# Shreyas2409/Rust-Image-Transform

Measured on AMD Instinct MI355X. Metric: transform MPix/s (decode+resize+encode) 4096²→512² WebP q80; 1/2/4/8 GPU, higher is better.
Workload: dtype u8

## Files before the change

rust-image-transform_amd/csrc/ik_png.hip:

```cpp
#include <algorithm>
#include <cstdlib>
#include <cstring>
#include <type_traits>

#include "ik_crc.h"
#include "ik_inflate.h"
#include "ik_internal.h"
#include "ik_png.h"
#include "ik_png_wave.h"
#include "ik_unfilter.h"

namespace ik {

__device__ __forceinline__ void raise_priority() { __builtin_amdgcn_s_setprio(3); }

typedef __attribute__((address_space(3))) uint32_t lds_word;
struct FindWin {
    const IK_GLOBAL uint32_t* W;
    uint64_t wend;
    lds_word* win;
    uint32_t r0;
    __device__ void fetch(uint64_t base) {
        if (base + 32 > wend + 64) {
            for (int k = 0; k < 32; ++k) win[64 * k] = base + k < wend ? W[base + k] : 0u;
// ... 1294 lines not shown
                const int i = __builtin_ctz(mk);
                mk &= mk - 1u;
                if (k < (uint32_t)kResolveList) {
                    s_pos[k++] = (uint32_t)(x0 + i);
                    continue;
                }
                const int rv = infl::resolve_at(I.u16, I.obase, I.nlanes, I.page_lane, kPngPageShift, e0 + i);
                if (rv < 0) atomicOr(err + ir.x, 2);
                o[i >> 2] = (o[i >> 2] & ~(255u << (8 * (i & 3)))) | (((uint32_t)rv & 255u) << (8 * (i & 3)));
            }
        }
        *reinterpret_cast<IK_GLOBAL uint4*>(drow + x0) = make_uint4(o[0], o[1], o[2], o[3]);
    }
    __syncthreads();
    const uint32_t cnt = s_cnt < (uint32_t)kResolveList ? s_cnt : (uint32_t)kResolveList;
    const int64_t hlo = s_hlo, hhi = s_hhi;
    for (uint32_t m = threadIdx.x; m < cnt; m += 256) {
        const uint32_t x = s_pos[m];
        const int64_t q = rs + 1 + (int64_t)x;
        int rv;
        if (q >= hlo && q < hhi) {
            const uint32_t mv = I.u16[q];
            const int64_t q2 = hlo - infl::kWindow + (int64_t)(mv & 0x7FFFu);
            rv = (mv & 0x8000u) && q2 >= 0 ? infl::resolve_at(I.u16, I.obase, I.nlanes, I.page_lane, kPngPageShift, q2) : -1;
        } else {
            rv = infl::resolve_at(I.u16, I.obase, I.nlanes, I.page_lane, kPngPageShift, q);
        }
        if (rv < 0) atomicOr(err + ir.x, 2);
        drow[x] = (uint8_t)rv;
    }
}

__device__ __forceinline__ uint32_t wave_shr1(uint32_t v, uint32_t lane0) {
    return (uint32_t)__builtin_amdgcn_update_dpp((int)lane0, (int)v, 0x138, 0xF, 0xF, false);
}

__device__ __forceinline__ uint32_t byte_of(const uint32_t (&w)[4], int i) { return (w[i >> 2] >> (8 * (i & 3))) & 255u; }

typedef unsigned u32x4 __attribute__((ext_vector_type(4)));
constexpr int kUnfG = 8;

typedef const __attribute__((address_space(1))) u32x4* gu32x4p;
constexpr int kCpolSc1 = 16;

__device__ __forceinline__ uint64_t uniform_u64(uint64_t v) {
    const uint32_t lo = (uint32_t)__builtin_amdgcn_readfirstlane((int)(uint32_t)v);
    const uint32_t hi = (uint32_t)__builtin_amdgcn_readfirstlane((int)(uint32_t)(v >> 32));
    return ((uint64_t)hi << 32) | lo;
}

struct FtMask {
    uint32_t sub, up, avg, paeth;
    __device__ explicit FtMask(uint32_t ft)
        : sub(ft == 1 ? ~0u : 0u), up(ft == 2 ? ~0u : 0u), avg(ft == 3 ? ~0u : 0u), paeth(ft == 4 ? ~0u : 0u) {}
};

template <int BPP, bool SWAR = false>
__device__ __forceinline__ void unfilter_chunk(const u32x4& rawv, const uint32_t (&up)[4], const uint32_t (&prevup)[4],
                                               const uint32_t (&prevcur)[4], const FtMask& fm, uint32_t (&o)[4]) {
    const uint32_t raw[4] = {rawv.x, rawv.y, rawv.z, rawv.w};
    if constexpr (SWAR && (BPP == 4 || BPP == 8)) {
        constexpr int K = BPP / 4;
#pragma unroll
        for (int k = 0; k < 4; ++k) {
            const uint32_t a = k >= K ? o[k - K] : prevcur[4 + k - K];
            const uint32_t c = k >= K ? up[k - K] : prevup[4 + k - K];
            o[k] = unfilter_word(raw[k], a, up[k], c, fm.sub, fm.up, fm.avg, fm.paeth);
        }
        return;
    }
    o[0] = o[1] = o[2] = o[3] = 0;
#pragma unroll
    for (int i = 0; i < 16; ++i) {
        const uint32_t a = i >= BPP ? ((o[(i - BPP) >> 2] >> (8 * ((i - BPP) & 3))) & 255u)
                                    : byte_of(prevcur, 16 + i - BPP);
        const uint32_t b = byte_of(up, i);
        const uint32_t c = i >= BPP ? byte_of(up, i - BPP) : byte_of(prevup, 16 + i - BPP);
        const int d1 = (int)b - (int)c, d2 = (int)a - (int)c;
        const int pa = d1 < 0 ? -d1 : d1, pb = d2 < 0 ? -d2 : d2, pc = (d1 + d2) < 0 ? -(d1 + d2) : (d1 + d2);
        const uint32_t paeth = (pa <= pb && pa <= pc) ? a : (pb <= pc ? b : c);
        const uint32_t pred = (a & fm.sub) | (b & fm.up) | (((a + b) >> 1) & fm.avg) | (paeth & fm.paeth);
        const uint32_t v = (byte_of(raw, i) + pred) & 255u;
        o[i >> 2] |= v << (8 * (i & 3));
    }
}

#ifdef IK_UNF_PROF
__device__ unsigned long long g_unf_prof[8];
hipError_t png_unf_prof_read(unsigned long long* out) {
    hipError_t e = hipMemcpyFromSymbol(out, HIP_SYMBOL(g_unf_prof), sizeof(g_unf_prof));
    unsigned long long z[8] = {};
    if (e == hipSuccess) e = hipMemcpyToSymbol(HIP_SYMBOL(g_unf_prof), z, sizeof(z));
    return e;
}
#define IK_UNF_T(k) do { const unsigned long long _t = clock64(); up_[k] += _t - t_; t_ = _t; } while (0)
#else
#define IK_UNF_T(k) do { } while (0)
#endif

template <int BPP, bool SWAR>
__global__ __launch_bounds__(kPngUnfilterThreads) void k_png_unfilter(const PngImgDev* imgs, const int2* groups,
                                                                      const int* prog_base, unsigned* prog,
                                                                      unsigned* ticket) {
    raise_priority();
    constexpr int NW = kPngUnfilterThreads / 64, G = kUnfG;
    __shared__ int s_t;
    if (threadIdx.x == 0) s_t = (int)atomicAdd(ticket, 1u);
    __syncthreads();
    const int2 gk = groups[s_t];
    const PngImgDev I = imgs[gk.x];
    if (png_unfilter_scan_path(BPP, I.rowbytes, *(const volatile int*)I.flags)) return;
    const int wave = __builtin_amdgcn_readfirstlane(threadIdx.x >> 6), lane = threadIdx.x & 63;
    const int nch = (I.rowbytes + 15) >> 4;
    const int nbands = (I.H + 63) >> 6;
    const int K = png_unfilter_groups(I.H);
    unsigned* pg = prog + prog_base[gk.x];
#ifdef IK_UNF_PROF
    unsigned long long up_[6] = {0, 0, 0, 0, 0, 0}, t_ = clock64();
#endif
    for (int band = wave * K + gk.y; band < nbands; band += NW * K) {
        const int y = band * 64 + lane;
        const bool live = y < I.H;
        const FtMask fm(live ? I.ft[y] : 0u);
        const bool above = band > 0;
        uint32_t cur[4] = {0, 0, 0, 0}, up[4] = {0, 0, 0, 0};
        uint32_t prevcur[4] = {0, 0, 0, 0}, prevup[4] = {0, 0, 0, 0};
        const uint64_t dbase = uniform_u64((uint64_t)(size_t)I.dst);
        const size_t ibytes = I.pitch * (size_t)I.H;
        const __amdgpu_buffer_rsrc_t rs = __builtin_amdgcn_make_buffer_rsrc(
            (void*)dbase, (short)0, (int)(ibytes < 0x7fffffffu ? ibytes : 0x7fffffffu), 0x00020000);
        const uint32_t rowoff = (uint32_t)((size_t)(live ? y : 0) * I.pitch);
        auto fetch = [&](int s0, u32x4 (&r)[G]) {
#pragma unroll
            for (int t = 0; t < G; ++t) {
                const uint32_t off = rowoff + 16u * (uint32_t)min(max(s0 + t - lane, 0), nch - 1);
                r[t] = __builtin_bit_cast(u32x4, __builtin_amdgcn_raw_buffer_load_b128(rs, (int)off, 0, 0));
            }
        };
        unsigned seen = 0;
        const int ngrp = (nch + 63 + G - 1) / G;
        auto group = [&](int g, u32x4 (&rc)[G], u32x4 (&rn)[G]) {
            const int s0 = g * G;
            u32x4 ab[G];
#pragma unroll
            for (int t = 0; t < G; ++t) ab[t] = u32x4{0, 0, 0, 0};
            IK_UNF_T(0);
            if (above && s0 < nch) {
                const unsigned need = (unsigned)min(s0 + G, nch);
                while (seen < need) {
                    const unsigned v = __hip_atomic_load(pg + band - 1, __ATOMIC_RELAXED, __HIP_MEMORY_SCOPE_AGENT);
                    seen = (unsigned)__builtin_amdgcn_readfirstlane((int)v);
                    if (seen < need) __builtin_amdgcn_s_sleep(1);
                }
                const uint32_t aoff = lane == 0 ? (uint32_t)((size_t)(band * 64 - 1) * I.pitch) : 0x80000000u;
#pragma unroll
                for (int t = 0; t < G; ++t)
                    ab[t] = __builtin_bit_cast(u32x4, __builtin_amdgcn_raw_buffer_load_b128(
                                                          rs, (int)(aoff + 16u * (uint32_t)min(s0 + t, nch - 1)), 0, kCpolSc1));
            }
            IK_UNF_T(1);
            if (g + 1 < ngrp) fetch(s0 + G, rn);
#pragma unroll
            for (int t = 0; t < G; ++t) {
                const int j = s0 + t - lane;
                uint32_t nup[4];
                nup[0] = wave_shr1(cur[0], ab[t].x);
                nup[1] = wave_shr1(cur[1], ab[t].y);
                nup[2] = wave_shr1(cur[2], ab[t].z);
                nup[3] = wave_shr1(cur[3], ab[t].w);
                const bool act = live && j >= 0 && j < nch;
                if (act) {
#pragma unroll
                    for (int k = 0; k < 4; ++k) { prevup[k] = up[k]; up[k] = nup[k]; prevcur[k] = cur[k]; }
                    if (j == 0) {
#pragma unroll
                        for (int k = 0; k < 4; ++k) { prevup[k] = 0; prevcur[k] = 0; }
                    }
                    uint32_t o[4];
                    unfilter_chunk<BPP, SWAR>(rc[t], up, prevup, prevcur, fm, o);
#pragma unroll
                    for (int k = 0; k < 4; ++k) cur[k] = o[k];
                }
                const u32x4 ov = {cur[0], cur[1], cur[2], cur[3]};
                __builtin_amdgcn_raw_buffer_store_b128(__builtin_bit_cast(__attribute__((ext_vector_type(4))) unsigned, ov),
                                                       rs, (int)(act ? rowoff + 16u * (uint32_t)j : 0x80000000u), 0,
                                                       kCpolSc1);
            }
            IK_UNF_T(2);
            const int jl = s0 + G - 1 - 63;
            if (jl >= 0 && band * 64 + 63 < I.H) {
                asm volatile("s_waitcnt vmcnt(0)" ::: "memory");
                if (lane == 63)
                    __hip_atomic_store(pg + band, (unsigned)min(jl + 1, nch), __ATOMIC_RELAXED, __HIP_MEMORY_SCOPE_AGENT);
            }
            IK_UNF_T(3);
        };
        u32x4 ra[G], rb[G];
        fetch(0, ra);
        for (int g = 0; g < ngrp; g += 2) {
            group(g, ra, rb);
            if (g + 1 < ngrp) group(g + 1, rb, ra);
        }
    }
#ifdef IK_UNF_PROF
    if (lane == 0) {
        for (int k = 0; k < 5; ++k) atomicAdd(&g_unf_prof[k], up_[k]);
        atomicAdd(&g_unf_prof[7], 1ull);
    }
#endif
}

__device__ __forceinline__ uint32_t add_bytes(uint32_t a, uint32_t b) {
    return ((a & 0x7F7F7F7Fu) + (b & 0x7F7F7F7Fu)) ^ ((a ^ b) & 0x80808080u);
}
__device__ __forceinline__ uint32_t wave_scan_bytes(uint32_t v) {
    v = add_bytes(v, (uint32_t)__builtin_amdgcn_update_dpp(0, (int)v, 0x111, 0xF, 0xF, true));
    v = add_bytes(v, (uint32_t)__builtin_amdgcn_update_dpp(0, (int)v, 0x112, 0xF, 0xF, true));
    v = add_bytes(v, (uint32_t)__builtin_amdgcn_update_dpp(0, (int)v, 0x114, 0xF, 0xF, true));
    v = add_bytes(v, (uint32_t)__builtin_amdgcn_update_dpp(0, (int)v, 0x118, 0xF, 0xF, true));
    const uint32_t r0 = (uint32_t)__builtin_amdgcn_readlane((int)v, 15);
    const uint32_t r1 = add_bytes(r0, (uint32_t)__builtin_amdgcn_readlane((int)v, 31));
    const uint32_t r2 = add_bytes(r1, (uint32_t)__builtin_amdgcn_readlane((int)v, 47));
    const int row = (int)(threadIdx.x & 63) >> 4;
    return add_bytes(v, row == 0 ? 0u : row == 1 ? r0 : row == 2 ? r1 : r2);
}

template <int CH>
__global__ __launch_bounds__(kSuThreads) void k_png_unfilter_su(const PngImgDev* imgs, int nimg) {
    raise_priority();
    constexpr int kSuChunks = CH;
    __shared__ uint32_t s_w[kSuThreads / 64];
    typedef uint32_t u4 __attribute__((ext_vector_type(4)));
    const int im = (int)blockIdx.x / kSuRanges, jr = (int)blockIdx.x % kSuRanges;
    if (im >= nimg) return;
    const PngImgDev I = imgs[im];
    if (!png_unfilter_scan_path(4, I.rowbytes, *(const volatile int*)I.flags)) return;
    const int H = I.H, nch = (I.rowbytes + 15) >> 4;
    if ((nch <= kSuThreads * ::ik::kSuChunks) != (CH == ::ik::kSuChunks)) return;
    const int tid = threadIdx.x, wv = tid >> 6;
    const int c0 = tid * kSuChunks;
    const int y1 = (int)((int64_t)H * (jr + 1) / kSuRanges);
    int y = (int)((int64_t)H * jr / kSuRanges);
    const IK_GLOBAL uint8_t* ft = (const IK_GLOBAL uint8_t*)I.ft;
    while (y < y1 && y != 0 && ft[y] > 1) ++y;
    while (y < y1) {
        uint32_t prev[4 * kSuChunks];
#pragma unroll
        for (int k = 0; k < 4 * kSuChunks; ++k) prev[k] = 0;
        int r = y;
        do {
            const uint32_t f = ft[r];
            IK_GLOBAL uint8_t* row = (IK_GLOBAL uint8_t*)(I.dst + (size_t)r * I.pitch);
            uint32_t w[4 * kSuChunks];
#pragma unroll
            for (int i = 0; i < kSuChunks; ++i) {
                const u4 v = c0 + i < nch ? *(const IK_GLOBAL u4*)(row + 16 * (c0 + i)) : u4{0, 0, 0, 0};
                w[4 * i] = v.x; w[4 * i + 1] = v.y; w[4 * i + 2] = v.z; w[4 * i + 3] = v.w;
            }
            if (f == 2) {
#pragma unroll
                for (int k = 0; k < 4 * kSuChunks; ++k) w[k] = add_bytes(w[k], prev[k]);
            } else if (f == 1) {
#pragma unroll
                for (int k = 1; k < 4 * kSuChunks; ++k) w[k] = add_bytes(w[k], w[k - 1]);
                const uint32_t incl = wave_scan_bytes(w[4 * kSuChunks - 1]);
                uint32_t carry = (uint32_t)__builtin_amdgcn_update_dpp(0, (int)incl, 0x138, 0xF, 0xF, true);
                if ((tid & 63) == 63) s_w[wv] = incl;
                __syncthreads();
                for (int q = 0; q < wv; ++q) carry = add_bytes(carry, s_w[q]);
                __syncthreads();
#pragma unroll
                for (int k = 0; k < 4 * kSuChunks; ++k) w[k] = add_bytes(w[k], carry);
            }
#pragma unroll
            for (int i = 0; i < kSuChunks; ++i)
                if (c0 + i < nch) *(IK_GLOBAL u4*)(row + 16 * (c0 + i)) = u4{w[4 * i], w[4 * i + 1], w[4 * i + 2], w[4 * i + 3]};
#pragma unroll
            for (int k = 0; k < 4 * kSuChunks; ++k) prev[k] = w[k];
            ++r;
        } while (r < H && ft[r] == 2);
        y = r;
    }
}

hipError_t launch_png_unfilter_su(const PngImgDev* imgs, int nimg, hipStream_t s) {
    if (nimg <= 0) return hipSuccess;
    hipLaunchKernelGGL(k_png_unfilter_su<kSuChunks>, dim3(nimg * kSuRanges), dim3(kSuThreads), 0, s, imgs, nimg);
    hipLaunchKernelGGL(k_png_unfilter_su<kSuChunksWide>, dim3(nimg * kSuRanges), dim3(kSuThreads), 0, s, imgs, nimg);
    return hipGetLastError();
}

__global__ __launch_bounds__(256) void k_copy_words(const uint32_t* __restrict__ src, uint32_t* __restrict__ dst,
                                                    size_t n) {
    for (size_t i = (size_t)blockIdx.x * 256 + threadIdx.x; i < n; i += (size_t)gridDim.x * 256) dst[i] = src[i];
}

hipError_t launch_copy_words(const uint32_t* src, uint32_t* dst, size_t n, hipStream_t s) {
    if (!n) return hipSuccess;
    const size_t blocks = std::min<size_t>((n + 255) / 256, 1024);
    hipLaunchKernelGGL(k_copy_words, dim3((unsigned)blocks), dim3(256), 0, s, src, dst, n);
    return hipGetLastError();
}

struct CrcOps {
    uint32_t x2n[32];
    uint32_t level[8];
    uint32_t piece;
    uint32_t crc_idat;
};

__global__ __launch_bounds__(256) void k_png_gather(uintptr_t raw, uint8_t* __restrict__ stream,
                                                    const PngGatherPiece* __restrict__ pieces,
                                                    uint32_t* __restrict__ piece_crc, CrcOps ops) {
    __shared__ uint32_t t[1024];
    __shared__ uint32_t s_crc[256], s_len[256];
    const int tid = (int)threadIdx.x;
    t[tid] = crc::table_entry((uint32_t)tid);
    __syncthreads();
#pragma unroll
    for (int sl = 1; sl < 4; ++sl) {
        const uint32_t prev = t[256 * (sl - 1) + tid];
        t[256 * sl + tid] = (prev >> 8) ^ t[prev & 255u];
        __syncthreads();
    }
    const PngGatherPiece P = pieces[blockIdx.x];
    const uint32_t b0 = 256u * (uint32_t)tid;
    const uint32_t len = P.len > b0 ? (P.len - b0 < 256u ? P.len - b0 : 256u) : 0u;
    uint32_t c = ~0u;
    IK_GLOBAL uint8_t* dp = (IK_GLOBAL uint8_t*)(stream + P.dst + b0);
    if (len && P.src == kPngNoSrc) {
        for (uint32_t i = 0; i < len; ++i) dp[i] = 0;
    } else if (len) {
        const IK_GLOBAL uint8_t* sp = (const IK_GLOBAL uint8_t*)(raw + (uintptr_t)(P.src + b0));
        uint32_t i = 0;
        const uint32_t mis = (uint32_t)((uintptr_t)dp & 3u);
        const uint32_t pre = mis ? (4u - mis < len ? 4u - mis : len) : 0u;
        for (; i < pre; ++i) {
            const uint32_t b = sp[i];
            dp[i] = (uint8_t)b;
            c = crc::step_byte(c, b, t);
        }
        const uint32_t nw = (len - i) >> 2;
        if (nw) {
            const uintptr_t sa = (uintptr_t)(sp + i);
            const uint32_t sh = (uint32_t)(sa & 3u);
            const IK_GLOBAL uint32_t* ws = reinterpret_cast<const IK_GLOBAL uint32_t*>(sa - sh);
            IK_GLOBAL uint32_t* wd = reinterpret_cast<IK_GLOBAL uint32_t*>(dp + i);
            uint32_t lo = ws[0];
            uint32_t k = 0;
            for (; k + 8 <= nw; k += 8) {
                uint32_t in[9];
                in[0] = lo;
#pragma unroll
                for (int u = 1; u <= 8; ++u) in[u] = sh ? ws[k + u] : (u < 8 ? ws[k + u] : 0u);
#pragma unroll
                for (int u = 0; u < 8; ++u) {
                    const uint32_t v = sh ? __builtin_amdgcn_alignbyte(in[u + 1], in[u], sh) : in[u];
                    wd[k + u] = v;
                    c = crc::step_word(c, v, t);
                }
                lo = sh ? in[8] : (k + 8 < nw ? ws[k + 8] : 0u);
            }
            for (; k < nw; ++k) {
                const uint32_t hi = sh ? ws[k + 1] : 0u;
                const uint32_t v = sh ? __builtin_amdgcn_alignbyte(hi, lo, sh) : lo;
                wd[k] = v;
                c = crc::step_word(c, v, t);
                lo = sh ? hi : (k + 1 < nw ? ws[k + 1] : 0u);
            }
            i += 4u * nw;
        }
        for (; i < len; ++i) {
            const uint32_t b = sp[i];
            dp[i] = (uint8_t)b;
            c = crc::step_byte(c, b, t);
        }
    }
    s_crc[tid] = ~c;
    s_len[tid] = len;
    __syncthreads();
#pragma unroll 1
    for (int k = 0; k < 8; ++k) {
        const int stride = 1 << k;
        if ((tid & (2 * stride - 1)) == 0) {
            const uint32_t rl = s_len[tid + stride];
            if (rl) {
                const uint32_t op = rl == (256u << k) ? ops.level[k] : crc::x8n(rl, ops.x2n);
                s_crc[tid] = crc::combine_op(s_crc[tid], s_crc[tid + stride], op);
                s_len[tid] += rl;
            }
        }
        __syncthreads();
    }
    if (tid == 0) {
        piece_crc[2 * blockIdx.x] = s_crc[0];
        piece_crc[2 * blockIdx.x + 1] = s_len[0];
    }
}

__global__ __launch_bounds__(256) void k_png_crc_check(uintptr_t raw,
                                                       const PngCrcChunk* __restrict__ chunks, int nchunks,
                                                       const uint32_t* __restrict__ piece_crc, int* err, CrcOps ops) {
    const int i = (int)(blockIdx.x * blockDim.x + threadIdx.x);
    if (i >= nchunks) return;
    const PngCrcChunk C = chunks[i];
    uint32_t c = ops.crc_idat;
    for (uint32_t p = C.piece0; p < C.piece0 + C.npieces; ++p) {
        const uint32_t len = piece_crc[2 * p + 1];
        const uint32_t op = len == kPngGatherPiece ? ops.piece : crc::x8n(len, ops.x2n);
        c = crc::combine_op(c, piece_crc[2 * p], op);
    }
    const IK_GLOBAL uint8_t* q = (const IK_GLOBAL uint8_t*)(raw + (uintptr_t)C.crc_at);
    const uint32_t stored = (uint32_t)q[0] << 24 | (uint32_t)q[1] << 16 | (uint32_t)q[2] << 8 | (uint32_t)q[3];
    if (c != stored) err[C.stream] = 1;
}

static CrcOps crc_ops() {
    static const CrcOps o = [] {
        CrcOps r{};
        crc::x2n_table(r.x2n);
        for (int k = 0; k < 8; ++k) r.level[k] = crc::x8n((uint64_t)256 << k, r.x2n);
        r.piece = crc::x8n(kPngGatherPiece, r.x2n);
        uint32_t t[1024];
        for (uint32_t i = 0; i < 256; ++i) t[i] = crc::table_entry(i);
        for (int sl = 1; sl < 4; ++sl)
            for (int i = 0; i < 256; ++i) t[256 * sl + i] = (t[256 * (sl - 1) + i] >> 8) ^ t[t[256 * (sl - 1) + i] & 255u];
        uint32_t c = ~0u;
        for (const char ch : {'I', 'D', 'A', 'T'}) c = crc::step_byte(c, (uint8_t)ch, t);
        r.crc_idat = ~c;
        return r;
    }();
    return o;
}

hipError_t launch_png_gather(uintptr_t raw, uint8_t* stream, const PngGatherPiece* pieces, int npieces,
                             uint32_t* piece_crc, hipStream_t s) {
    if (npieces <= 0) return hipSuccess;
    hipLaunchKernelGGL(k_png_gather, dim3((unsigned)npieces), dim3(256), 0, s, raw, stream, pieces, piece_crc,
                       crc_ops());
    return hipGetLastError();
}

hipError_t launch_png_crc_check(uintptr_t raw, const PngCrcChunk* chunks, int nchunks, const uint32_t* piece_crc,
                                int* err, hipStream_t s) {
    if (nchunks <= 0) return hipSuccess;
    hipLaunchKernelGGL(k_png_crc_check, dim3((unsigned)((nchunks + 255) / 256)), dim3(256), 0, s, raw, chunks,
                       nchunks, piece_crc, err, crc_ops());
    return hipGetLastError();
}

__global__ __launch_bounds__(64) void k_png_walk(const uint64_t* __restrict__ files, const uint64_t* __restrict__ lens,
                                                 PngWalkRec* __restrict__ recs, uint8_t* __restrict__ side,
                                                 int* __restrict__ out_n) {
    const int f = (int)blockIdx.x, lane = (int)threadIdx.x;
    const IK_GLOBAL uint8_t* b = (const IK_GLOBAL uint8_t*)(uintptr_t)files[f];
    const uint64_t n = lens[f];
    PngWalkRec* R = recs + (size_t)f * kPngWalkRecs;
    uint8_t* S = side + (size_t)f * kPngWalkSide;
    uint64_t pos = 8;
    uint32_t used = 0;
    int cnt = 0, st = 0;
    while (pos + 12 <= n) {
        uint8_t h[12];
#pragma unroll
        for (int k = 0; k < 12; ++k) h[k] = b[pos + k];
        const uint32_t len = (uint32_t)h[0] << 24 | (uint32_t)h[1] << 16 | (uint32_t)h[2] << 8 | h[3];
        if ((uint64_t)len > n - pos - 12) { st = -3; break; }
        if (cnt == kPngWalkRecs) { st = -1; break; }
        const bool idat = h[4] == 'I' && h[5] == 'D' && h[6] == 'A' && h[7] == 'T';
        uint32_t so = ~0u;
        if (!idat || !len) {
            if (used + len + 8 > kPngWalkSide) { st = -2; break; }
            so = used;
            for (uint32_t i = (uint32_t)lane; i < len + 8; i += 64) S[so + i] = b[pos + 4 + i];
            used += (len + 8 + 3) & ~3u;
        }
        if (lane == 0) {
            PngWalkRec r;
            r.off = pos;
            r.len = len;
            r.side = so;
#pragma unroll
            for (int k = 0; k < 4; ++k) { r.type[k] = h[4 + k]; r.head[k] = h[8 + k]; }
            R[cnt] = r;
        }
        ++cnt;
        pos += 12 + (uint64_t)len;
        if (h[4] == 'I' && h[5] == 'E' && h[6] == 'N' && h[7] == 'D') break;
    }
    if (lane == 0) out_n[f] = st ? st : cnt;
}

__global__ __launch_bounds__(64) void k_copy_heads(const uint64_t* __restrict__ files, const uint64_t* __restrict__ lens,
                                                   uint8_t* __restrict__ out) {
    const int f = (int)blockIdx.x, t = (int)threadIdx.x;
    const IK_GLOBAL uint8_t* b = (const IK_GLOBAL uint8_t*)(uintptr_t)files[f];
    out[64 * (size_t)f + t] = (uint64_t)t < lens[f] ? b[t] : 0;
}

hipError_t launch_copy_heads(const uint64_t* files, const uint64_t* lens, int n, uint8_t* out, hipStream_t s) {
    if (n <= 0) return hipSuccess;
    hipLaunchKernelGGL(k_copy_heads, dim3((unsigned)n), dim3(64), 0, s, files, lens, out);
    return hipGetLastError();
}

hipError_t launch_png_walk(const uint64_t* files, const uint64_t* lens, int n, PngWalkRec* recs, uint8_t* side,
                           int* out_n, hipStream_t s) {
    if (n <= 0) return hipSuccess;
    hipLaunchKernelGGL(k_png_walk, dim3((unsigned)n), dim3(64), 0, s, files, lens, recs, side, out_n);
    return hipGetLastError();
}

__device__ __forceinline__ int a7_pass(uint32_t xr, int yr) {
    if (yr & 1) return 6;
    if (xr & 1) return 5;
    if (yr & 2) return 4;
    if (xr & 2) return 3;
    if (yr & 4) return 2;
    return (xr & 4) ? 1 : 0;
}

template <int BITS>
__device__ __forceinline__ void a7_row(const PngA7Dev& I, int y, uint32_t seg, uint8_t* lds) {
    constexpr int UB = BITS == 24 || BITS == 48 ? 48 : 16;
    constexpr uint32_t SEG = kA7Threads * UB;
    typedef uint32_t u4 __attribute__((ext_vector_type(4)));
    const uint32_t tid = threadIdx.x;
    const size_t ub = (size_t)seg * SEG + (size_t)tid * UB;
    IK_GLOBAL uint8_t* const drow = (IK_GLOBAL uint8_t*)(I.dst + (size_t)y * I.pitch);
    if (y & 1) {
        const IK_GLOBAL uint8_t* srow = (const IK_GLOBAL uint8_t*)(I.pass[6].src + (size_t)(y >> 1) * I.pass[6].pitch);
#pragma unroll
        for (int c = 0; c < UB / 16; ++c)
            if (ub + 16 * c < (size_t)I.rowbytes) *(IK_GLOBAL u4*)(drow + ub + 16 * c) = *(const IK_GLOBAL u4*)(srow + ub + 16 * c);
        return;
    }
    const int yr = y & 7;
#pragma unroll
    for (int p = 0; p < 6; ++p) {
        const int ldx = 3 - (p >> 1), ldy = p < 3 ? 3 : p < 5 ? 2 : 1, y0 = p == 2 ? 4 : p == 4 ? 2 : 0;
        if ((yr - y0) & ((1 << ldy) - 1)) continue;
        const uint32_t len = SEG >> ldx, ro = (p & 1) ? len : 0u;
        const size_t s0 = ((size_t)seg * SEG) >> ldx;
        const IK_GLOBAL uint8_t* srow = (const IK_GLOBAL uint8_t*)(I.pass[p].src + (size_t)(y >> ldy) * I.pass[p].pitch);
        for (uint32_t b = tid * 16; b < len; b += kA7Threads * 16) {
            u4 v = {0, 0, 0, 0};
            if (I.pass[p].src && s0 + b < (size_t)I.pass[p].rowbytes) v = *(const IK_GLOBAL u4*)(srow + s0 + b);
            *reinterpret_cast<u4*>(lds + ro + b) = v;
        }
    }
    __syncthreads();
    uint32_t o[UB / 4];
#pragma unroll
    for (int k = 0; k < UB / 4; ++k) o[k] = 0;
    if constexpr (BITS >= 8) {
        constexpr int BPP = BITS / 8, NPX = UB / BPP;
        constexpr int E = BPP % 4 == 0 ? 4 : BPP % 2 == 0 ? 2 : 1;
#pragma unroll
        for (int i = 0; i < NPX; ++i) {
            const uint32_t xl = tid * NPX + i;
            const int p = a7_pass(xl & 7u, yr), ldx = 3 - (p >> 1);
            const uint32_t a = ((p & 1) ? SEG >> ldx : 0u) + (xl >> ldx) * BPP;
#pragma unroll
            for (int k = 0; k < BPP / E; ++k) {
                const int pos = i * BPP + k * E;
                uint32_t v;
                if constexpr (E == 4) v = *reinterpret_cast<const uint32_t*>(lds + a + 4 * k);
                else if constexpr (E == 2) v = *reinterpret_cast<const uint16_t*>(lds + a + 2 * k);
                else v = lds[a + k];
                o[pos >> 2] |= v << (8 * (pos & 3));
            }
        }
    } else {
        constexpr int F = 8 / BITS;
#pragma unroll
        for (int j = 0; j < 16; ++j) {
            uint32_t byte = 0;
#pragma unroll
            for (int f = 0; f < F; ++f) {
                const uint32_t xl = (tid * 16 + j) * F + f;
                const int p = a7_pass(xl & 7u, yr), ldx = 3 - (p >> 1);
                const uint32_t sb = (xl >> ldx) * BITS;
                const uint32_t v = ((uint32_t)lds[((p & 1) ? SEG >> ldx : 0u) + (sb >> 3)] >> (8 - BITS - (sb & 7u))) & ((1u << BITS) - 1u);
                byte |= v << (8 - BITS - f * BITS);
            }
            o[j >> 2] |= byte << (8 * (j & 3));
        }
    }
#pragma unroll
    for (int c = 0; c < UB / 16; ++c)
        if (ub + 16 * c < (size_t)I.rowbytes)
            *(IK_GLOBAL u4*)(drow + ub + 16 * c) = u4{o[4 * c], o[4 * c + 1], o[4 * c + 2], o[4 * c + 3]};
}

__global__ __launch_bounds__(kA7Threads) void k_png_adam7(const PngA7Dev* imgs, int n) {
    raise_priority();
    __shared__ __attribute__((aligned(16))) uint8_t s_run[kA7Threads * 48];
    int lo = 0, hi = n - 1;
    while (lo < hi) {
        const int mid = (lo + hi + 1) >> 1;
        if (imgs[mid].blk0 <= blockIdx.x) lo = mid;
        else hi = mid - 1;
    }
    const PngA7Dev& I = imgs[lo];
    const uint32_t r = blockIdx.x - I.blk0;
    const int y = (int)(r / I.nseg);
    const uint32_t seg = r % I.nseg;
    if (y >= I.h) return;
    switch (I.bits) {
    case 1: a7_row<1>(I, y, seg, s_run); break;
    case 2: a7_row<2>(I, y, seg, s_run); break;
    case 4: a7_row<4>(I, y, seg, s_run); break;
    case 8: a7_row<8>(I, y, seg, s_run); break;
    case 16: a7_row<16>(I, y, seg, s_run); break;
    case 24: a7_row<24>(I, y, seg, s_run); break;
    case 32: a7_row<32>(I, y, seg, s_run); break;
    case 48: a7_row<48>(I, y, seg, s_run); break;
    case 64: a7_row<64>(I, y, seg, s_run); break;
    default: break;
    }
}

hipError_t launch_png_adam7(const PngA7Dev* imgs, int n, uint32_t nblocks, hipStream_t s) {
    if (n <= 0 || !nblocks) return hipSuccess;
    hipLaunchKernelGGL(k_png_adam7, dim3(nblocks), dim3(kA7Threads), 0, s, imgs, n);
    return hipGetLastError();
}

__global__ __launch_bounds__(256) void k_png_px(PngPxDev P) {
    __shared__ uint32_t pal[256];
    if (P.ctype == 3) pal[threadIdx.x] = P.pal[threadIdx.x];
    __syncthreads();
    const int x = (int)(blockIdx.x * 256 + threadIdx.x), y = (int)blockIdx.y;
    if (x >= P.w) return;
    const uint8_t* r = P.src + (size_t)y * P.sp;
    if (P.depth == 16) {
        const int spp = P.ctype == 0 ? 1 : P.ctype == 2 ? 3 : P.ctype == 4 ? 2 : 4;
        const uint8_t* s = r + (size_t)2 * spp * x;
        uint16_t* o16 = reinterpret_cast<uint16_t*>(P.dst + (size_t)y * P.dp) + (size_t)x * P.out_c;
        bool key = P.out_c > spp;
#pragma unroll 4
        for (int k = 0; k < spp; ++k) {
            const int v = (int)s[2 * k] << 8 | s[2 * k + 1];
            o16[k] = (uint16_t)v;
            key = key && v == (P.ctype == 0 ? P.key : P.key_rgb[k]);
        }
        if (P.out_c > spp) o16[spp] = key ? 0 : 65535;
        return;
    }
    uint8_t* o = P.dst + (size_t)y * P.dp + (size_t)x * P.out_c;
    if (P.ctype == 2) {
        const int R = r[3 * x], G = r[3 * x + 1], B = r[3 * x + 2];
        o[0] = (uint8_t)R; o[1] = (uint8_t)G; o[2] = (uint8_t)B;
        o[3] = (R == P.key_rgb[0] && G == P.key_rgb[1] && B == P.key_rgb[2]) ? 0 : 255;
        return;
    }
    int v;
    if (P.depth == 8) {
        v = r[x];
    } else {
        const int bit = x * P.depth;
        v = (r[bit >> 3] >> (8 - P.depth - (bit & 7))) & ((1 << P.depth) - 1);
    }
    if (P.ctype == 3) {
        const uint32_t c = pal[v];
        o[0] = (uint8_t)c; o[1] = (uint8_t)(c >> 8); o[2] = (uint8_t)(c >> 16);
        if (P.out_c == 4) o[3] = (uint8_t)(c >> 24);
    } else {
        o[0] = (uint8_t)(v * P.scale);
        if (P.out_c == 2) o[1] = v == P.key ? 0 : 255;
    }
}

hipError_t launch_png_px(const PngPxDev& px, hipStream_t s) {
    if (px.w <= 0 || px.h <= 0) return hipSuccess;
    hipLaunchKernelGGL(k_png_px, dim3((unsigned)((px.w + 255) / 256), (unsigned)px.h), dim3(256), 0, s, px);
    return hipGetLastError();
}

hipError_t launch_png_find(const PngImgDev* imgs, const int* chunk_img, const int* chunk_idx, int n,
                           uint64_t chunk_bits, int64_t* cand, hipStream_t s) {
    if (n <= 0) return hipSuccess;
    hipLaunchKernelGGL(k_png_find, dim3(n), dim3(64), 0, s, imgs, chunk_img, chunk_idx, n, chunk_bits, cand);
    return hipGetLastError();
}

hipError_t launch_png_decode(const PngImgDev* imgs, const PngLaneDev* lanes, const uint32_t* order, int n,
                             uint16_t* tok, infl::LaneResult* res, hipStream_t s) {
    if (n <= 0) return hipSuccess;
    const dim3 grid((n + kPngInflateThreads - 1) / kPngInflateThreads);
    hipLaunchKernelGGL(k_png_decode, grid, dim3(kPngInflateThreads), 0, s, imgs, lanes, order, n, tok, res);
    return hipGetLastError();
}

hipError_t launch_png_marks(const PngImgDev* imgs, PngMarks mk, const int2* rows, int nrows, int* err, hipStream_t s) {
    hipLaunchKernelGGL(k_png_marks, dim3(8 * kMarkLists), dim3(256), 0, s, imgs, mk, err);
    if (nrows > 0) hipLaunchKernelGGL(k_png_ftflags, dim3((nrows + 255) / 256), dim3(256), 0, s, imgs, rows, nrows, err);
    return hipGetLastError();
}

hipError_t launch_png_expand(const PngImgDev* imgs, const PngLaneDev* lanes, int n, const uint16_t* tok, int* status,
                             hipStream_t s, const uint2* pieces, const uint2* units, const uint32_t* ulane, PngMarks mk) {
    if (n <= 0) return hipSuccess;
    if ((units != nullptr) != (ulane != nullptr) || (units && !pieces)) return hipErrorInvalidValue;
    if (mk.list && !pieces) return hipErrorInvalidValue;
    if (pieces)
        hipLaunchKernelGGL(k_png_expand8<false>, dim3(n), dim3(64), 0, s, imgs, lanes, n, tok, status, pieces, units, ulane, mk);
    else
        hipLaunchKernelGGL(k_png_expand8<true>, dim3(n), dim3(64), 0, s, imgs, lanes, n, tok, status, pieces, units, ulane, mk);
    return hipGetLastError();
}

hipError_t launch_png_wave(const PngImgDev* imgs, const PngLaneDev* lanes, const uint32_t* order, int n,
                           uint16_t* tok, uint2* pieces, uint2* units, infl::LaneResult* res, hipStream_t s) {
    if (n <= 0) return hipSuccess;
    hipLaunchKernelGGL(k_png_wave, dim3(n), dim3(64), 0, s, imgs, lanes, order, n, tok, pieces, units, res);
    return hipGetLastError();
}

hipError_t launch_png_units(const PngImgDev* imgs, const PngLaneDev* lanes, int n, const uint2* units,
                            uint32_t* ulane, hipStream_t s) {
    if (n <= 0) return hipSuccess;
    hipLaunchKernelGGL(k_png_units, dim3((n + 255) / 256), dim3(256), 0, s, imgs, lanes, n, units, ulane);
    return hipGetLastError();
}

hipError_t launch_png_resolve(const PngImgDev* imgs, const int2* rows, int nrows, int* err, hipStream_t s) {
    if (nrows <= 0) return hipSuccess;
    const dim3 grid(nrows < 65535 ? nrows : 65535, (nrows + 65534) / 65535);
    hipLaunchKernelGGL(k_png_resolve, grid, dim3(256), 0, s, imgs, rows, nrows, err);
    return hipGetLastError();
}

hipError_t launch_png_unfilter(const PngImgDev* imgs, const int2* groups, int ngroups, const int* prog_base,
                               unsigned* prog, unsigned* ticket, int bpp, hipStream_t s) {
    if (ngroups <= 0) return hipSuccess;
    const dim3 grid(ngroups), block(kPngUnfilterThreads);
#define IK_UNF(B, W) hipLaunchKernelGGL((k_png_unfilter<B, W>), grid, block, 0, s, imgs, groups, prog_base, prog, ticket)
    switch (bpp) {
    case 1: IK_UNF(1, false); break;
    case 2: IK_UNF(2, false); break;
    case 3: IK_UNF(3, false); break;
// ... 11 lines not shown
```

Baseline: 31330.

## Rewrite PNG IDAT gather with 16-byte interleaved copy and GF(2) CRC combining

The PNG IDAT gather kernel no longer gives each thread a serial 256-byte run. Threads now each handle interleaved 16-byte granules using vector loads and stores, realign them across lanes with DPP shifts, and compute per-thread partial CRCs. The partials are combined with precomputed GF(2) multipliers and a wave-level xor reduction, replacing the log-step tree combine. A persistent grid of 512-thread blocks loops over pieces instead of launching one block per piece. This targets better memory coalescing and more parallel CRC work, at the cost of per-block polynomial-multiply setup and complex edge masking that is easy to get wrong.

```diff
diff --git a/rust-image-transform_amd/csrc/ik_png.hip b/rust-image-transform_amd/csrc/ik_png.hip
--- a/rust-image-transform_amd/csrc/ik_png.hip
+++ b/rust-image-transform_amd/csrc/ik_png.hip
@@ -1620,99 +1620,179 @@
     return hipGetLastError();
 }
 
+constexpr int kGatherThreads = 512;
+constexpr uint32_t kGatherRow = 16u * kGatherThreads;
+constexpr int kGatherGrid = 1024;
+
 struct CrcOps {
     uint32_t x2n[32];
-    uint32_t level[8];
+    uint32_t gran[9];
+    uint32_t row;
+    uint32_t pre[16];
+    uint32_t unpad[16];
     uint32_t piece;
     uint32_t crc_idat;
 };
 
-__global__ __launch_bounds__(256) void k_png_gather(uintptr_t raw, uint8_t* __restrict__ stream,
-                                                    const PngGatherPiece* __restrict__ pieces,
-                                                    uint32_t* __restrict__ piece_crc, CrcOps ops) {
-    __shared__ uint32_t t[1024];
-    __shared__ uint32_t s_crc[256], s_len[256];
-    const int tid = (int)threadIdx.x;
-    t[tid] = crc::table_entry((uint32_t)tid);
+__device__ __forceinline__ uint32_t crc_mul(uint32_t a, uint32_t b) {
+    uint32_t p = 0;
+#pragma unroll
+    for (int i = 31; i >= 0; --i) {
+        p ^= (uint32_t)((int32_t)(a << (31 - i)) >> 31) & b;
+        b = (b >> 1) ^ ((0u - (b & 1u)) & crc::kPoly);
+    }
+    return p;
+}
+
+typedef uint32_t gather_u4 __attribute__((ext_vector_type(4)));
+
+__device__ __forceinline__ void gather_store(uintptr_t oa, gather_u4 v, uintptr_t da, uintptr_t de) {
+    if (oa >= da && oa + 16 <= de) {
+        *reinterpret_cast<IK_GLOBAL gather_u4*>(oa) = v;
+        return;
+    }
+    const uint32_t w[4] = {v.x, v.y, v.z, v.w};
+#pragma unroll
+    for (int i = 0; i < 16; ++i)
+        if (oa + i >= da && oa + i < de) *reinterpret_cast<IK_GLOBAL uint8_t*>(oa + i) = (uint8_t)(w[i >> 2] >> (8 * (i & 3)));
+}
+
+__global__ __launch_bounds__(kGatherThreads) void k_png_gather(uintptr_t raw, uint8_t* __restrict__ stream,
+                                                               const PngGatherPiece* __restrict__ pieces, int npieces,
+                                                               uint32_t* __restrict__ piece_crc, CrcOps ops) {
+    typedef gather_u4 u4;
+    __shared__ uint32_t s_t[1024];
+    __shared__ uint32_t s_k[1024];
+    __shared__ uint32_t s_part[2][kGatherThreads / 64];
+    static_assert(sizeof(s_t) + sizeof(s_k) + sizeof(s_part) <= 7 * 1280 && 7 * 4 < 5 * (kGatherThreads / 64),
+                  "k_png_gather's LDS: 7 units per 8 waves, under the 5 units per 4 waves it had");
+    static_assert(kGatherRow == 8192 && kGatherThreads == 512, "CrcOps::row and ::gran are made for this geometry");
+    const uint32_t tid = threadIdx.x, lane = tid & 63u, wave = tid >> 6;
+    if (tid < 256) s_t[tid] = crc::table_entry(tid);
     __syncthreads();
 #pragma unroll
     for (int sl = 1; sl < 4; ++sl) {
-        const uint32_t prev = t[256 * (sl - 1) + tid];
-        t[256 * sl + tid] = (prev >> 8) ^ t[prev & 255u];
+        if (tid < 256) {
+            const uint32_t prev = s_t[256 * (sl - 1) + tid];
+            s_t[256 * sl + tid] = (prev >> 8) ^ s_t[prev & 255u];
+        }
         __syncthreads();
     }
-    const PngGatherPiece P = pieces[blockIdx.x];
-    const uint32_t b0 = 256u * (uint32_t)tid;
-    const uint32_t len = P.len > b0 ? (P.len - b0 < 256u ? P.len - b0 : 256u) : 0u;
-    uint32_t c = ~0u;
-    IK_GLOBAL uint8_t* dp = (IK_GLOBAL uint8_t*)(stream + P.dst + b0);
-    if (len && P.src == kPngNoSrc) {
-        for (uint32_t i = 0; i < len; ++i) dp[i] = 0;
-    } else if (len) {
-        const IK_GLOBAL uint8_t* sp = (const IK_GLOBAL uint8_t*)(raw + (uintptr_t)(P.src + b0));
-        uint32_t i = 0;
-        const uint32_t mis = (uint32_t)((uintptr_t)dp & 3u);
-        const uint32_t pre = mis ? (4u - mis < len ? 4u - mis : len) : 0u;
-        for (; i < pre; ++i) {
-            const uint32_t b = sp[i];
-            dp[i] = (uint8_t)b;
-            c = crc::step_byte(c, b, t);
-        }
-        const uint32_t nw = (len - i) >> 2;
-        if (nw) {
-            const uintptr_t sa = (uintptr_t)(sp + i);
-            const uint32_t sh = (uint32_t)(sa & 3u);
-            const IK_GLOBAL uint32_t* ws = reinterpret_cast<const IK_GLOBAL uint32_t*>(sa - sh);
-            IK_GLOBAL uint32_t* wd = reinterpret_cast<IK_GLOBAL uint32_t*>(dp + i);
-            uint32_t lo = ws[0];
-            uint32_t k = 0;
-            for (; k + 8 <= nw; k += 8) {
-                uint32_t in[9];
-                in[0] = lo;
-#pragma unroll
-                for (int u = 1; u <= 8; ++u) in[u] = sh ? ws[k + u] : (u < 8 ? ws[k + u] : 0u);
-#pragma unroll
-                for (int u = 0; u < 8; ++u) {
-                    const uint32_t v = sh ? __builtin_amdgcn_alignbyte(in[u + 1], in[u], sh) : in[u];
-                    wd[k + u] = v;
-                    c = crc::step_word(c, v, t);
+    {
+        const uint32_t q = 3u - (tid >> 8), i = tid & 255u;
+        uint32_t v = crc_mul(ops.row, i << (8 * q));
+        s_k[256 * q + i] = v;
+        v = (v >> 8) ^ s_t[v & 255u];
+        v = (v >> 8) ^ s_t[v & 255u];
+        s_k[256 * (q - 2) + i] = v;
+    }
+    uint32_t wgt = crc::kOne;
+#pragma unroll 1
+    for (int b = 0; b < 9; ++b)
+        if ((tid >> b) & 1u) wgt = crc_mul(ops.gran[b], wgt);
+    __syncthreads();
+
+    uint32_t joins = 0;
+    for (int p = (int)blockIdx.x; p < npieces; p += (int)gridDim.x) {
+        const PngGatherPiece P = pieces[p];
+        const uint32_t len = P.len;
+        const uintptr_t da = (uintptr_t)stream + (uintptr_t)P.dst, de = da + len;
+        if (len == 0 || P.src == kPngNoSrc) {
+            if (len) {
+                const uintptr_t d0 = da & ~(uintptr_t)15;
+                const uint32_t n = (uint32_t)((((de - 1) & ~(uintptr_t)15) - d0) >> 4) + 1u;
+                for (uint32_t k = tid; k < n; k += kGatherThreads) gather_store(d0 + 16u * (uintptr_t)k, u4{0, 0, 0, 0}, da, de);
+            }
+            if (tid == 0) {
+                piece_crc[2 * (size_t)p] = 0;
+                piece_crc[2 * (size_t)p + 1] = len;
+            }
+            continue;
+        }
+        const uintptr_t sa = raw + (uintptr_t)P.src;
+        const uintptr_t s_first = sa & ~(uintptr_t)15, s_last = (sa + len - 1) & ~(uintptr_t)15;
+        const uint32_t h = (uint32_t)(sa & 15u);
+        const uint32_t u = 15u - (uint32_t)((sa + len - 1) & 15u);
+        const uint32_t ngran = (uint32_t)((s_last - s_first) >> 4) + 1u;
+        const uint32_t s = (uint32_t)((sa - da) & 15u);
+        const uint32_t nk = ngran + (s ? 1u : 0u);
+        const uintptr_t o_last = s_last + s + da - sa;
+        const uint32_t pre = ops.pre[h];
+        const int rows = (int)((nk + kGatherThreads - 1) / kGatherThreads);
+
+        auto load = [&](uint32_t k) -> u4 {
+            return k < ngran ? *reinterpret_cast<const IK_GLOBAL u4*>(s_last - 16u * (uintptr_t)k) : u4{0, 0, 0, 0};
+        };
+        auto load_edge = [&](uint32_t k) -> u4 {
+            return (s && lane == 0 && k >= 1u) ? load(k - 1u) : u4{0, 0, 0, 0};
+        };
+        uint32_t S = 0;
+        uint32_t k = tid + kGatherThreads * (uint32_t)(rows - 1);
+        u4 cur = load(k), edge = load_edge(k);
+        for (int j = rows - 1; j >= 0; --j, k -= kGatherThreads) {
+            u4 nxt{0, 0, 0, 0}, nedge{0, 0, 0, 0};
+            if (j > 0) {
+                nxt = load(k - kGatherThreads);
+                nedge = load_edge(k - kGatherThreads);
+            }
+            if (k - lane < nk) {
+                u4 out = cur;
+                if (s) {
+                    uint32_t w[8] = {cur.x, cur.y, cur.z, cur.w, 0, 0, 0, 0};
+                    w[4] = (uint32_t)__builtin_amdgcn_update_dpp((int)edge.x, (int)cur.x, 0x138, 0xF, 0xF, false);
+                    w[5] = (uint32_t)__builtin_amdgcn_update_dpp((int)edge.y, (int)cur.y, 0x138, 0xF, 0xF, false);
+                    w[6] = (uint32_t)__builtin_amdgcn_update_dpp((int)edge.z, (int)cur.z, 0x138, 0xF, 0xF, false);
+                    w[7] = (uint32_t)__builtin_amdgcn_update_dpp((int)edge.w, (int)cur.w, 0x138, 0xF, 0xF, false);
+                    uint32_t v[5];
+                    switch (s >> 2) {
+                        case 0: v[0] = w[0], v[1] = w[1], v[2] = w[2], v[3] = w[3], v[4] = w[4]; break;
+                        case 1: v[0] = w[1], v[1] = w[2], v[2] = w[3], v[3] = w[4], v[4] = w[5]; break;
+                        case 2: v[0] = w[2], v[1] = w[3], v[2] = w[4], v[3] = w[5], v[4] = w[6]; break;
+                        default: v[0] = w[3], v[1] = w[4], v[2] = w[5], v[3] = w[6], v[4] = w[7]; break;
+                    }
+                    const uint32_t r = s & 3u;
+                    out.x = __builtin_amdgcn_alignbyte(v[1], v[0], r);
+                    out.y = __builtin_amdgcn_alignbyte(v[2], v[1], r);
+                    out.z = __builtin_amdgcn_alignbyte(v[3], v[2], r);
+                    out.w = __builtin_amdgcn_alignbyte(v[4], v[3], r);
                 }
-                lo = sh ? in[8] : (k + 8 < nw ? ws[k + 8] : 0u);
-            }
-            for (; k < nw; ++k) {
-                const uint32_t hi = sh ? ws[k + 1] : 0u;
-                const uint32_t v = sh ? __builtin_amdgcn_alignbyte(hi, lo, sh) : lo;
-                wd[k] = v;
-                c = crc::step_word(c, v, t);
-                lo = sh ? hi : (k + 1 < nw ? ws[k + 1] : 0u);
-            }
-            i += 4u * nw;
-        }
-        for (; i < len; ++i) {
-            const uint32_t b = sp[i];
-            dp[i] = (uint8_t)b;
-            c = crc::step_byte(c, b, t);
-        }
-    }
-    s_crc[tid] = ~c;
-    s_len[tid] = len;
-    __syncthreads();
-#pragma unroll 1
-    for (int k = 0; k < 8; ++k) {
-        const int stride = 1 << k;
-        if ((tid & (2 * stride - 1)) == 0) {
-            const uint32_t rl = s_len[tid + stride];
-            if (rl) {
-                const uint32_t op = rl == (256u << k) ? ops.level[k] : crc::x8n(rl, ops.x2n);
-                s_crc[tid] = crc::combine_op(s_crc[tid], s_crc[tid + stride], op);
-                s_len[tid] += rl;
-            }
-        }
+                if (k < nk) gather_store(o_last - 16u * (uintptr_t)k, out, da, de);
+                u4 g = cur;
+                if (k == 0 || k + 1u == ngran) {
+                    const uint32_t lo = k + 1u == ngran ? h : 0u, hi = k == 0 ? 16u - u : 16u;
+                    uint32_t m[4];
+#pragma unroll
+                    for (uint32_t i = 0; i < 4; ++i) {
+                        const uint32_t a = lo > 4 * i ? (lo >= 4 * i + 4 ? 0u : ~0u << (8 * (lo - 4 * i))) : ~0u;
+                        const uint32_t b = hi < 4 * i + 4 ? (hi <= 4 * i ? 0u : ~0u >> (8 * (4 * i + 4 - hi))) : ~0u;
+                        m[i] = a & b;
+                    }
+                    g.x &= m[0], g.y &= m[1], g.z &= m[2], g.w &= m[3];
+                }
+                uint32_t c = k + 1u == ngran ? pre : 0u;
+                c = crc::step_word(c, g.x, s_t);
+                c = crc::step_word(c, g.y, s_t);
+                c = crc::step_word(c, g.z, s_t);
+                c = crc::step_word(c, g.w, s_t);
+                S = s_k[S & 255u] ^ s_k[256 + ((S >> 8) & 255u)] ^ s_k[512 + ((S >> 16) & 255u)] ^ s_k[768 + (S >> 24)] ^ c;
+            }
+            cur = nxt;
+            edge = nedge;
+        }
+        uint32_t x = crc_mul(wgt, S);
+#pragma unroll
+        for (int m = 32; m >= 1; m >>= 1) x ^= (uint32_t)__shfl_xor((int)x, m);
+        uint32_t* part = s_part[joins & 1u];
+        ++joins;
+        if (lane == 0) part[wave] = x;
         __syncthreads();
-    }
-    if (tid == 0) {
-        piece_crc[2 * blockIdx.x] = s_crc[0];
-        piece_crc[2 * blockIdx.x + 1] = s_len[0];
+        if (tid == 0) {
+            uint32_t t = 0;
+#pragma unroll
+            for (int i = 0; i < kGatherThreads / 64; ++i) t ^= part[i];
+            piece_crc[2 * (size_t)p] = ~crc_mul(ops.unpad[u], t);
+            piece_crc[2 * (size_t)p + 1] = len;
+        }
     }
 }
 
@@ -1737,7 +1817,12 @@
     static const CrcOps o = [] {
         CrcOps r{};
         crc::x2n_table(r.x2n);
-        for (int k = 0; k < 8; ++k) r.level[k] = crc::x8n((uint64_t)256 << k, r.x2n);
+        for (int b = 0; b < 9; ++b) r.gran[b] = crc::x8n((uint64_t)16 << b, r.x2n);
+        r.row = crc::x8n(kGatherRow, r.x2n);
+        for (uint32_t n = 0; n < 16; ++n) {
+            r.unpad[n] = crc::x8n(0xFFFFFFFFull - n, r.x2n);
+            r.pre[n] = crc::multmodp(r.unpad[n], 0xFFFFFFFFu);
+        }
         r.piece = crc::x8n(kPngGatherPiece, r.x2n);
         uint32_t t[1024];
         for (uint32_t i = 0; i < 256; ++i) t[i] = crc::table_entry(i);
@@ -1754,8 +1839,8 @@
 hipError_t launch_png_gather(uintptr_t raw, uint8_t* stream, const PngGatherPiece* pieces, int npieces,
                              uint32_t* piece_crc, hipStream_t s) {
     if (npieces <= 0) return hipSuccess;
-    hipLaunchKernelGGL(k_png_gather, dim3((unsigned)npieces), dim3(256), 0, s, raw, stream, pieces, piece_crc,
-                       crc_ops());
+    hipLaunchKernelGGL(k_png_gather, dim3((unsigned)std::min(npieces, kGatherGrid)), dim3(kGatherThreads), 0, s, raw,
+                       stream, pieces, npieces, piece_crc, crc_ops());
     return hipGetLastError();
 }
 
```

Measured after the change: 32230, median of 6. 2.9% higher.
